# idiap/IdiapTTS

Hardware: AMD Instinct MI355X
Metric: acoustic frames/sec (train) (higher is better)
Workload: dtype f32

## Files before the change

### idiaptts_amd/csrc/sparse_rows.hip

```cpp
#include <algorithm>
#include <atomic>
#include <utility>

#include "activations.h"
#include "common.h"
#include "dropout.h"

namespace itts {

constexpr int kSparseMaxK = 512;
constexpr int kSlabCols = 64;
constexpr int kFwdWaves = 16;
constexpr int kRowsPerWave = 4;
constexpr int kStep = 8;
constexpr int kFetch = 16;
constexpr int kFillTrips = kSparseMaxK / 4 / kFwdWaves;

static std::atomic<int64_t> g_sparse_path[3];

struct ListLayout {
  int64_t counts_off, entries_off, pitch, bytes;
};

static ListLayout list_layout(int64_t M, int K) {
  ListLayout l;
  l.counts_off = 16;
  l.entries_off = 16 + (M * 4 + 15) / 16 * 16;
  l.pitch = ((int64_t)K + kFetch - 1) / kFetch * kFetch;
  l.bytes = l.entries_off + M * l.pitch * 8;
  return l;
}

__global__ __launch_bounds__(256) void sparse_rows_build_kernel(const uint32_t* __restrict__ x, int64_t ldx, int64_t M,
                                                                int K, int* __restrict__ counts,
                                                                int2* __restrict__ entries, int64_t pitch,
                                                                unsigned long long* __restrict__ record) {
  const int lane = threadIdx.x & 63;
  const int64_t w0 = (int64_t)blockIdx.x * 4 + (threadIdx.x >> 6), wn = (int64_t)gridDim.x * 4;
  const unsigned long long below = (1ull << lane) - 1ull;
  unsigned long long total = 0, most = 0;
  for (int64_t m = w0; m < M; m += wn) {
    const uint32_t* row = x + m * ldx;
    int2* out = entries + m * pitch;
    int cnt = 0;
    for (int k0 = 0; k0 < K; k0 += 256) {
      uint32_t bits[4];
#pragma unroll
      for (int u = 0; u < 4; ++u) {
        const int k = k0 + 64 * u + lane;
        bits[u] = k < K ? row[k] : 0u;
      }
#pragma unroll
      for (int u = 0; u < 4; ++u) {
        const bool nz = (bits[u] & 0x7fffffffu) != 0u;
        const unsigned long long mask = __ballot(nz);
        if (nz) out[cnt + __popcll(mask & below)] = make_int2(k0 + 64 * u + lane, (int)bits[u]);
        cnt += __popcll(mask);
      }
    }
    if (lane < ((kStep - cnt % kStep) % kStep)) out[cnt + lane] = make_int2(K, 0);
    if (lane == 0) counts[m] = cnt;
    total += (unsigned long long)cnt;
    most = std::max(most, (unsigned long long)cnt);
  }
  if (record && lane == 0 && total) {
    atomicAdd(&record[0], total);
    atomicMax(&record[1], most);
  }
}

template <int J>
__device__ __forceinline__ void walk_slot(const float4* slab4, int i16, int2 e, float4& acc) {
  const int k = __builtin_amdgcn_update_dpp(0, e.x, 0x150 + J, 0xf, 0xf, false);
  const float v = __int_as_float(__builtin_amdgcn_update_dpp(0, e.y, 0x150 + J, 0xf, 0xf, false));
  const float4 wk = slab4[k * (kSlabCols / 4) + i16];
  acc.x = fmaf(v, wk.x, acc.x); acc.y = fmaf(v, wk.y, acc.y);
  acc.z = fmaf(v, wk.z, acc.z); acc.w = fmaf(v, wk.w, acc.w);
}
template <int FIRST, int... U>
__device__ __forceinline__ void walk_trip(const float4* slab4, int i16, int2 e, float4& acc,
                                          std::integer_sequence<int, U...>) {
  (walk_slot<FIRST + U>(slab4, i16, e, acc), ...);
}

template <int AF, class DR = NoDrop>
__global__ __launch_bounds__(kFwdWaves * 64) void sparse_linear_fwd_kernel(
    const int* __restrict__ counts, const int2* __restrict__ entries, int64_t pitch, const float* __restrict__ w,
    const float* __restrict__ bias, float* __restrict__ y, int64_t ldy, int64_t M, int N, int K, int act, int ranges,
    int store_cols, int wide_out, int wide_w, DR dr) {
  extern __shared__ float4 slab4[];
  float* slab = reinterpret_cast<float*>(slab4);
  const int lane = threadIdx.x & 63;
  const int wave = __builtin_amdgcn_readfirstlane((int)(threadIdx.x >> 6));
  const int n0 = (int)(blockIdx.x / ranges) * kSlabCols;
  const int range = (int)(blockIdx.x % ranges);
  const int64_t per = (M + ranges - 1) / ranges;
  const int64_t m_begin = range * per, m_end = std::min<int64_t>(M, m_begin + per);
  const int q = lane >> 4, c4 = (lane & 15) * 4;

  {
    const bool col_ok = n0 + lane < N;
    const float* wr = w + (int64_t)(col_ok ? n0 + lane : 0) * K;
    if (wide_w) {
      const float4* wr4 = reinterpret_cast<const float4*>(wr);
      const int K4 = K >> 2;
      float4 v[kFillTrips];
#pragma unroll
      for (int u = 0; u < kFillTrips; ++u) {
        const int j = wave + u * kFwdWaves;
        v[u] = (col_ok && j < K4) ? wr4[j] : make_float4(0.f, 0.f, 0.f, 0.f);
      }
#pragma unroll
      for (int u = 0; u < kFillTrips; ++u) {
        const int j = wave + u * kFwdWaves;
        if (j < K4) {
          float* row = slab + 4 * j * kSlabCols + lane;
          row[0] = v[u].x; row[kSlabCols] = v[u].y; row[2 * kSlabCols] = v[u].z; row[3 * kSlabCols] = v[u].w;
        }
      }
    } else {
      for (int k = wave; k < K; k += kFwdWaves) slab[k * kSlabCols + lane] = col_ok ? wr[k] : 0.f;
    }
    if (wave == 0) slab[K * kSlabCols + lane] = 0.f;
  }

  auto row_of = [&](int64_t group) { return m_begin + (group * kRowsPerWave + q); };
  const int i16 = lane & 15;
  auto fetch = [&](int64_t m, int j0) { return entries[std::min<int64_t>(m, M - 1) * pitch + (j0 + i16)]; };
  int64_t group = wave;
  int2 first = fetch(row_of(group), 0);
  int cnt_next = counts[std::min<int64_t>(row_of(group), M - 1)];
  __syncthreads();

  float4 bv = make_float4(0.f, 0.f, 0.f, 0.f);
  const int n = n0 + c4;
  if (bias) {
    if (n < N) bv.x = bias[n];
    if (n + 1 < N) bv.y = bias[n + 1];
    if (n + 2 < N) bv.z = bias[n + 2];
    if (n + 3 < N) bv.w = bias[n + 3];
  }
  const bool vec_store = wide_out && n + 4 <= store_cols;
  const int last_fetch = (int)pitch - kFetch;

  for (; m_begin + group * kRowsPerWave < m_end; group += kFwdWaves) {
    const int64_t m = row_of(group);
    const int cnt = m < m_end ? cnt_next : 0;
    int2 cur = first;
    first = fetch(row_of(group + kFwdWaves), 0);
    cnt_next = counts[std::min<int64_t>(row_of(group + kFwdWaves), M - 1)];
    int longest = std::max(cnt, __shfl_xor(cnt, 16, 64));
    longest = __builtin_amdgcn_readfirstlane(std::max(longest, __shfl_xor(longest, 32, 64)));
    float4 acc = make_float4(0.f, 0.f, 0.f, 0.f);
    for (int j0 = 0; j0 < longest; j0 += kFetch) {
      const int2 nxt = fetch(m, std::min(j0 + kFetch, last_fetch));
      if (j0 < cnt) walk_trip<0>(slab4, i16, cur, acc, std::make_integer_sequence<int, kStep>());
      if (j0 + kStep < cnt) walk_trip<kStep>(slab4, i16, cur, acc, std::make_integer_sequence<int, kStep>());
      cur = nxt;
    }
    if (m < m_end) {
      float4 o;
      o.x = n < N ? act_fwd_af<AF>(acc.x + bv.x, act) : 0.f;
      o.y = n + 1 < N ? act_fwd_af<AF>(acc.y + bv.y, act) : 0.f;
      o.z = n + 2 < N ? act_fwd_af<AF>(acc.z + bv.z, act) : 0.f;
      o.w = n + 3 < N ? act_fwd_af<AF>(acc.w + bv.w, act) : 0.f;
      if constexpr (DR::on) {
        const uint4x dw = dr.words(m, n);
        o.x = dr.apply(o.x, dw.w[0]); o.y = dr.apply(o.y, dw.w[1]);
        o.z = dr.apply(o.z, dw.w[2]); o.w = dr.apply(o.w, dw.w[3]);
      }
      float* yr = y + m * ldy + n;
      if (vec_store) {
        *reinterpret_cast<float4*>(yr) = o;
      } else {
        if (n < store_cols) yr[0] = o.x;
        if (n + 1 < store_cols) yr[1] = o.y;
        if (n + 2 < store_cols) yr[2] = o.z;
        if (n + 3 < store_cols) yr[3] = o.w;
      }
    }
  }
}

}

using namespace itts;

extern "C" int itts_sparse_rows_layout(int64_t M, int K, int64_t out[4]) {
  ITTS_REQUIRE(out != nullptr, "null pointer");
  ITTS_REQUIRE(M >= 0 && K > 0 && K <= 65535, "bad sizes (K <= 65535)");
  const ListLayout l = list_layout(M, K);
  out[0] = l.counts_off; out[1] = l.entries_off; out[2] = l.pitch; out[3] = l.bytes;
  return ITTS_OK;
}

extern "C" int itts_sparse_rows_build(const float* d_x, int64_t ldx, int64_t M, int K, void* d_lists, int want_record,
                                      void* stream) {
  ITTS_REQUIRE(d_lists && (M == 0 || d_x), "null pointer");
  ITTS_REQUIRE(M >= 0 && K > 0 && K <= 65535 && ldx >= K, "bad sizes (K <= 65535)");
  ITTS_REQUIRE(aligned16(d_lists), "the list block must be 16-byte aligned");
  hipStream_t s = as_stream(stream);
  char* base = static_cast<char*>(d_lists);
  if (want_record) ITTS_HIP_CHECK(hipMemsetAsync(base, 0, 16, s));
  if (M == 0) return ITTS_OK;
  const ListLayout l = list_layout(M, K);
  const unsigned grid = (unsigned)std::min<int64_t>((M + 3) / 4, 8192);
  hipLaunchKernelGGL(sparse_rows_build_kernel, dim3(grid), dim3(256), 0, s, reinterpret_cast<const uint32_t*>(d_x), ldx,
                     M, K, reinterpret_cast<int*>(base + l.counts_off), reinterpret_cast<int2*>(base + l.entries_off),
                     l.pitch, want_record ? reinterpret_cast<unsigned long long*>(base) : nullptr);
  ITTS_LAUNCH_CHECK();
  g_sparse_path[0].fetch_add(1, std::memory_order_relaxed);
  return ITTS_OK;
}

static int fwd_compute_units() {
  static int cus = 0;
  if (cus == 0) {
    int dev = 0, n = 0;
    if (hipGetDevice(&dev) != hipSuccess ||
        hipDeviceGetAttribute(&n, hipDeviceAttributeMultiprocessorCount, dev) != hipSuccess || n <= 0)
      n = 256;
    cus = n;
  }
  return cus;
}

template <int AF, class DR = NoDrop>
static int launch_sparse_fwd(const void* d_lists, const float* d_w, const float* d_b, float* d_y, int64_t ldy, int64_t M,
                             int N, int K, int act, hipStream_t s, const DR& dr = DR()) {
  ITTS_HIP_CHECK(itts::allow_dynamic_lds((const void*)sparse_linear_fwd_kernel<AF, DR>, (kSparseMaxK + 1) * kSlabCols * 4));
  const ListLayout l = list_layout(M, K);
  const char* base = static_cast<const char*>(d_lists);
  const int slabs = (N + kSlabCols - 1) / kSlabCols;
  const int64_t ranges = std::max<int64_t>(1, std::min<int64_t>(fwd_compute_units() / slabs, (M + 63) / 64));
  const bool wide_out = (ldy % 4 == 0) && aligned16(d_y);
  const int store_cols = wide_out ? (int)std::min<int64_t>((N + 3) / 4 * 4, ldy) : N;
  hipLaunchKernelGGL((sparse_linear_fwd_kernel<AF, DR>), dim3((unsigned)(slabs * ranges)), dim3(kFwdWaves * 64),
                     (size_t)(K + 1) * kSlabCols * 4, s, reinterpret_cast<const int*>(base + l.counts_off),
                     reinterpret_cast<const int2*>(base + l.entries_off), l.pitch, d_w, d_b, d_y, ldy, M, N, K, act,
                     (int)ranges, store_cols, wide_out ? 1 : 0, (K % 4 == 0 && aligned16(d_w)) ? 1 : 0, dr);
  ITTS_LAUNCH_CHECK();
  return ITTS_OK;
}

template <class DR>
static int linear_fwd_sparse(const void* d_lists, const float* d_x, int64_t ldx, const float* d_w, const float* d_b,
                             float* d_y, int64_t ldy, int64_t M, int N, int K, int act, hipStream_t s, const DR& dr) {
  const char* const entry = DR::on ? "itts_linear_fwd_sparse_dropout" : "itts_linear_fwd_sparse";
  ITTS_REQUIRE_AS(entry, d_w && (M == 0 || (d_lists && d_x && d_y)), "null pointer");
  ITTS_REQUIRE_AS(entry, M >= 0 && N > 0 && K > 0 && K <= 65535 && ldx >= K && ldy >= N, "bad sizes");
  ITTS_REQUIRE_AS(entry, act >= ITTS_ACT_NONE && act <= ITTS_ACT_HARDSIGMOID, "unknown activation");
  if (M == 0) return ITTS_OK;
  if (K > kSparseMaxK) {
    g_sparse_path[2].fetch_add(1, std::memory_order_relaxed);
    return itts::linear_fwd(d_x, ldx, d_w, d_b, d_y, ldy, M, N, K, act, s, dr);
  }
  g_sparse_path[1].fetch_add(1, std::memory_order_relaxed);
  if (act_family(act) == AF_EXT) return launch_sparse_fwd<AF_EXT, DR>(d_lists, d_w, d_b, d_y, ldy, M, N, K, act, s, dr);
  return launch_sparse_fwd<AF_BASE, DR>(d_lists, d_w, d_b, d_y, ldy, M, N, K, act, s, dr);
}

extern "C" int itts_linear_fwd_sparse(const void* d_lists, const float* d_x, int64_t ldx, const float* d_w,
                                      const float* d_b, float* d_y, int64_t ldy, int64_t M, int N, int K, int act,
                                      void* stream) {
  return linear_fwd_sparse(d_lists, d_x, ldx, d_w, d_b, d_y, ldy, M, N, K, act, as_stream(stream), NoDrop{});
}

extern "C" int itts_linear_fwd_sparse_dropout(const void* d_lists, const float* d_x, int64_t ldx, const float* d_w,
                                              const float* d_b, float* d_y, int64_t ldy, int64_t M, int N, int K,
                                              int act, double p, uint64_t seed, uint32_t salt, int64_t row_offset,
                                              void* stream) {
  ITTS_REQUIRE_DROP_P(p);
  if (p == 0.0)
    return linear_fwd_sparse(d_lists, d_x, ldx, d_w, d_b, d_y, ldy, M, N, K, act, as_stream(stream), NoDrop{});
  return linear_fwd_sparse(d_lists, d_x, ldx, d_w, d_b, d_y, ldy, M, N, K, act, as_stream(stream),
                           make_drop_rule(p, seed, salt, row_offset));
}

extern "C" int itts_sparse_path_counts(int64_t out[3]) {
  ITTS_REQUIRE(out != nullptr, "null pointer");
  for (int i = 0; i < 3; ++i) out[i] = g_sparse_path[i].load(std::memory_order_relaxed);
  return ITTS_OK;
}
```

### idiaptts_amd/csrc/sparse_wgrad.hip

```cpp
#include <algorithm>
#include <atomic>

#include "common.h"

namespace itts {

constexpr int kWgMaxK = 512;
constexpr int kTile = 256;
constexpr int kSlab = 64;
constexpr int kWgWaves = 16;
constexpr int kOwners = 64;
constexpr int kSlots = 8;
constexpr int kStrip = 32;
constexpr int kBlock = 16;
constexpr int kGroup = 4;
constexpr int kHeaderBytes = kSlots * 2;
constexpr int kFirstBytes = kBlock * 8;
constexpr int kOverBytes = (kTile / kBlock - 1) * kBlock * 8;
constexpr int kPlanInv = kStrip + kOwners * kSlots;
constexpr int kPlanInts = kPlanInv + kWgMaxK;
constexpr int kHeavyCode = 0x1000;
constexpr int kRowBytes = kSlab * 4;
constexpr int kBufBytes = (kTile + 1) * kRowBytes;
constexpr int kTPitch = 513;
// ... 99 lines not shown
constexpr int kFromRowsLdsBytes = kLists * kFirstBytes + kTile * kStrip * 4 + kFromRowsWaves * kLists * 4 + kWgMaxK * 4;

__global__ __launch_bounds__(kFromRowsWaves * 64) void sparse_cols_from_rows_kernel(
    const int* __restrict__ counts, const int4* __restrict__ entries2, int64_t pitch2, int64_t M, int K, int tiles,
    const int* __restrict__ plan, uint32_t* __restrict__ strip, char* __restrict__ streams) {
  constexpr int T = kFromRowsWaves * 64;
  extern __shared__ uint4 from_rows_lds[];
  int2* first = reinterpret_cast<int2*>(from_rows_lds);
  uint32_t* tile_strip = reinterpret_cast<uint32_t*>(first + kLists * kBlock);
  uint32_t* words = tile_strip + kTile * kStrip;
  int* inverse = reinterpret_cast<int*>(words + kFromRowsWaves * kLists);
  const int tid = threadIdx.x, lane = tid & 63, l32 = lane & 31;
  const int wave = __builtin_amdgcn_readfirstlane(tid >> 6);
  const int tile = (int)blockIdx.x;
  const int64_t m0 = (int64_t)tile * kTile;
  const int row0 = wave * 2 * kFromRowsPairs + (lane >> 5);

  int code_of_tid = -1;
  if (tid < K) {
    const int code = plan[kPlanInv + tid];
    if ((code >= 0 && code < kLists) || (code >= kHeavyCode && code < kHeavyCode + kStrip - 1)) code_of_tid = code;
  }
  int cnt[kFromRowsPairs];
  int4 head[kFromRowsPairs];
#pragma unroll
  for (int q = 0; q < kFromRowsPairs; ++q) {
    const int64_t m = m0 + row0 + 2 * q;
    const bool in = m < M && l32 < pitch2;
    cnt[q] = in ? std::min(counts[m], (int)(2 * pitch2)) : 0;
    head[q] = in ? entries2[m * pitch2 + l32] : make_int4(-1, 0, -1, 0);
  }

  {
    const uint4 neutral = make_uint4((uint32_t)(kTile * kRowBytes), 0u, (uint32_t)(kTile * kRowBytes), 0u);
    uint4* first4 = reinterpret_cast<uint4*>(first);
    for (int i = tid; i < kLists * kFirstBytes / 16; i += T) first4[i] = neutral;
    uint4* strip4 = reinterpret_cast<uint4*>(tile_strip);
    for (int i = tid; i < kTile * kStrip / 4; i += T) {
      const bool ones = (i & 7) == 7 && m0 + (i >> 3) < M;
      strip4[i] = make_uint4(0u, 0u, 0u, ones ? 0x3f800000u : 0u);
    }
    uint4* words4 = reinterpret_cast<uint4*>(words);
    for (int i = tid; i < kFromRowsWaves * kLists / 4; i += T) words4[i] = make_uint4(0u, 0u, 0u, 0u);
    if (tid < kWgMaxK) inverse[tid] = code_of_tid;
  }
  int most = 0;
#pragma unroll
  for (int q = 0; q < kFromRowsPairs; ++q) {
    if (2 * l32 >= cnt[q]) head[q].x = -1;
    if (2 * l32 + 1 >= cnt[q]) head[q].z = -1;
    most = std::max(most, cnt[q]);
  }
  const bool further = std::max(most, __shfl_xor(most, 32, 64)) > 64;
  __syncthreads();

  uint32_t* my_words = words + wave * kLists;
  auto code_of = [&](int k) { return (unsigned)k < (unsigned)K ? inverse[k] : -1; };
  auto again = [&](int q, int j0) {
    int4 e = j0 + 2 * l32 < cnt[q] ? entries2[(m0 + row0 + 2 * q) * pitch2 + j0 / 2 + l32] : make_int4(-1, 0, -1, 0);
    if (j0 + 2 * l32 + 1 >= cnt[q]) e.z = -1;
    e.x = code_of(e.x);
    e.z = code_of(e.z);
    return e;
  };
  auto mark = [&](int q, int code) {
    if (code >= 0 && code < kLists) atomicOr(&my_words[code], 1u << (2 * q + (lane >> 5)));
  };
  auto place = [&](int q, int code, int value) {
    const int row = 2 * q + (lane >> 5);
    if (code >= 0 && code < kLists) {
      const uint32_t word = my_words[code];
      const int pos = (int)(word >> 16) + __popc(word & ((1u << row) - 1u));
      const int2 out = make_int2((row0 + 2 * q) * kRowBytes, value);
      if (pos < kBlock) first[code * kBlock + pos] = out;
      else if (pos < kTile) *entry_of(streams, tiles, (int64_t)tile * kLists + code, pos) = out;
    } else if (code >= kHeavyCode) {
      tile_strip[(row0 + 2 * q) * kStrip + (code - kHeavyCode)] = (uint32_t)value;
    }
  };

#pragma unroll
  for (int q = 0; q < kFromRowsPairs; ++q) {
    head[q].x = code_of(head[q].x);
    head[q].z = code_of(head[q].z);
  }
#pragma unroll
  for (int q = 0; q < kFromRowsPairs; ++q) {
    mark(q, head[q].x);
    mark(q, head[q].z);
  }
  if (further) {
#pragma unroll
    for (int q = 0; q < kFromRowsPairs; ++q)
      for (int j0 = 64; j0 < cnt[q]; j0 += 64) {
        const int4 e = again(q, j0);
        mark(q, e.x);
        mark(q, e.z);
      }
  }
  __syncthreads();

  if (tid < kLists) {
    int run = 0;
#pragma unroll
    for (int w = 0; w < kFromRowsWaves; ++w) {
      const uint32_t rows_of_wave = words[w * kLists + tid];
      words[w * kLists + tid] = rows_of_wave | ((uint32_t)run << 16);
      run += __popc(rows_of_wave);
    }
    reinterpret_cast<uint16_t*>(streams)[(int64_t)tile * kLists + tid] = (uint16_t)run;
  }
  __syncthreads();

#pragma unroll
  for (int q = 0; q < kFromRowsPairs; ++q) {
    place(q, head[q].x, head[q].y);
    place(q, head[q].z, head[q].w);
  }
  if (further) {
#pragma unroll
    for (int q = 0; q < kFromRowsPairs; ++q)
      for (int j0 = 64; j0 < cnt[q]; j0 += 64) {
        const int4 e = again(q, j0);
        place(q, e.x, e.y);
        place(q, e.z, e.w);
      }
  }
  __syncthreads();

  {
    const uint4* first4 = reinterpret_cast<const uint4*>(first);
    uint4* dst = reinterpret_cast<uint4*>(const_cast<char*>(firsts_of(streams, tiles)) +
                                          (int64_t)tile * kLists * kFirstBytes);
    for (int i = tid; i < kLists * kFirstBytes / 16; i += T) dst[i] = first4[i];
    const uint4* strip4 = reinterpret_cast<const uint4*>(tile_strip);
    uint4* sdst = reinterpret_cast<uint4*>(strip + m0 * kStrip);
    for (int i = tid; i < kTile * kStrip / 4; i += T) sdst[i] = strip4[i];
  }
  {
    const int list = tid & (kLists - 1);
    const uint32_t last = words[(kFromRowsWaves - 1) * kLists + list];
    const int total = (int)(last >> 16) + __popc(last & 0xffffu);
    if (total > kBlock) {
      const int end = (total + kBlock - 1) / kBlock * kBlock;
      for (int e = total + (tid >> 9); e < end; e += T / kLists)
        *entry_of(streams, tiles, (int64_t)tile * kLists + list, e) = make_int2(kTile * kRowBytes, 0);
    }
  }
}

typedef float floatx16 __attribute__((ext_vector_type(16)));

template <int J>
__device__ __forceinline__ void col_slot(const char* buf, int lane_off, int2 e, float4& acc) {
  const int off = __builtin_amdgcn_update_dpp(0, e.x, 0x150 + J, 0xf, 0xf, false);
  const float v = __int_as_float(__builtin_amdgcn_update_dpp(0, e.y, 0x150 + J, 0xf, 0xf, false));
  const float4 d = *reinterpret_cast<const float4*>(buf + off + lane_off);
  acc.x = fmaf(v, d.x, acc.x); acc.y = fmaf(v, d.y, acc.y);
  acc.z = fmaf(v, d.z, acc.z); acc.w = fmaf(v, d.w, acc.w);
}
template <int FIRST>
__device__ __forceinline__ void col_group(const char* buf, int lane_off, int2 e, float4& acc) {
  col_slot<FIRST>(buf, lane_off, e, acc);
  col_slot<FIRST + 1>(buf, lane_off, e, acc);
  col_slot<FIRST + 2>(buf, lane_off, e, acc);
  col_slot<FIRST + 3>(buf, lane_off, e, acc);
}

__global__ __launch_bounds__(kWgWaves * 64) void sparse_wgrad_kernel(
    const float* __restrict__ dz, int64_t lddz, const float* __restrict__ strip, const char* __restrict__ streams,
    const int* __restrict__ plan, float* __restrict__ slabs, int64_t slab_stride, int lddw,
    float* __restrict__ bias_part, int64_t bias_stride, int64_t M, int N, int K, int tiles, int per, int ranges) {
  extern __shared__ float4 smem4[];
  char* smem = reinterpret_cast<char*>(smem4);
  float* smemf = reinterpret_cast<float*>(smem4);
  const int tid = threadIdx.x, lane = tid & 63;
  const int wave = __builtin_amdgcn_readfirstlane(tid >> 6);
  const int i16 = lane & 15, owner = wave * 4 + (lane >> 4);
  const int n0 = (int)(blockIdx.x / ranges) * kSlab;
  const int range = (int)(blockIdx.x % ranges);
  const int t_begin = range * per, t_end = std::min(tiles, t_begin + per);

  if (tid < 128) smemf[((tid >> 6) * kBufBytes + kTile * kRowBytes) / 4 + lane] = 0.f;

  const int srow = tid >> 4, c4 = (tid & 15) * 4, n = n0 + c4;
  auto load_tile = [&](int t, float4 (&st)[4]) {
#pragma unroll
    for (int p = 0; p < 4; ++p) {
      const int64_t m = (int64_t)t * kTile + p * 64 + srow;
      float4 v = make_float4(0.f, 0.f, 0.f, 0.f);
      if (m < M) {
        const float* src = dz + m * lddz + n;
        if (n + 4 <= N) {
          v = *reinterpret_cast<const float4*>(src);
        } else {
          if (n < N) v.x = src[0];
          if (n + 1 < N) v.y = src[1];
          if (n + 2 < N) v.z = src[2];
        }
      }
      st[p] = v;
    }
  };
  auto store_tile = [&](int b, const float4 (&st)[4]) {
#pragma unroll
    for (int p = 0; p < 4; ++p)
      *reinterpret_cast<float4*>(smem + b * kBufBytes + (p * 64 + srow) * kRowBytes + c4 * 4) = st[p];
  };
  const char* firsts = firsts_of(streams, tiles) + i16 * 8;
  const char* overs = overs_of(streams, tiles) + i16 * 8;
  auto lists_of = [&](int t) { return ((int64_t)t * kOwners + owner) * kSlots; };

  float4 acc[kSlots];
#pragma unroll
  for (int c = 0; c < kSlots; ++c) acc[c] = make_float4(0.f, 0.f, 0.f, 0.f);
  floatx16 hacc;
#pragma unroll
  for (int r = 0; r < 16; ++r) hacc[r] = 0.f;

  uint4 hdr;
  int2 first[kSlots];
  auto load_lists = [&](int t) {
    hdr = *reinterpret_cast<const uint4*>(streams + ((int64_t)t * kOwners + owner) * kHeaderBytes);
#pragma unroll
    for (int c = 0; c < kSlots; ++c)
      first[c] = *reinterpret_cast<const int2*>(firsts + (lists_of(t) + c) * kFirstBytes);
  };
  auto count_of = [&](int c) {
    const uint32_t word = c < 2 ? hdr.x : (c < 4 ? hdr.y : (c < 6 ? hdr.z : hdr.w));
    return (int)((word >> ((c & 1) * 16)) & 0xffffu);
  };

  float4 st[4];
  load_tile(t_begin, st);
  load_lists(t_begin);
  store_tile(0, st);
  __syncthreads();

  const int hb = wave >> 3, hr0 = (wave & 7) * 32 + (lane >> 5);
  for (int t = t_begin; t < t_end; ++t) {
    const int b = (t - t_begin) & 1;
    const int tn = std::min(t + 1, t_end - 1);
    const char* buf = smem + b * kBufBytes;
    const char* more = overs + lists_of(t) * kOverBytes;
    int2 over = first[0];
    if (count_of(0) > kBlock) over = *reinterpret_cast<const int2*>(more);
#pragma unroll
    for (int c = 0; c < kSlots; ++c) {
      const int cnt = count_of(c);
      int longest = std::max(cnt, __shfl_xor(cnt, 16, 64));
      longest = __builtin_amdgcn_readfirstlane(std::max(longest, __shfl_xor(longest, 32, 64)));
      int2 over_n = over;
      if (c + 1 < kSlots && count_of(c + 1 < kSlots ? c + 1 : c) > kBlock)
        over_n = *reinterpret_cast<const int2*>(more + (c + 1) * kOverBytes);
      int2 cur = first[c];
      for (int j0 = 0; j0 < longest; j0 += kBlock) {
        const int left = cnt - j0;
        if (left > 0) {
          int2 ahead = over;
          if (left > 2 * kBlock) ahead = *reinterpret_cast<const int2*>(more + c * kOverBytes + (j0 + kBlock) * 8);
          col_group<0>(buf, i16 * 16, cur, acc[c]);
          if (left > kGroup) col_group<kGroup>(buf, i16 * 16, cur, acc[c]);
          if (left > 2 * kGroup) col_group<2 * kGroup>(buf, i16 * 16, cur, acc[c]);
          if (left > 3 * kGroup) col_group<3 * kGroup>(buf, i16 * 16, cur, acc[c]);
          cur = over;
          over = ahead;
        }
      }
      over = over_n;
    }
    load_tile(tn, st);
    {
      const float* a = reinterpret_cast<const float*>(buf) + hr0 * kSlab + hb * 32 + (lane & 31);
      const float* xh = strip + ((int64_t)t * kTile + hr0) * kStrip + (lane & 31);
#pragma unroll
      for (int kk = 0; kk < 16; ++kk)
        hacc = __builtin_amdgcn_mfma_f32_32x32x2f32(a[2 * kk * kSlab], xh[2 * kk * kStrip], hacc, 0, 0, 0);
    }
    store_tile(b ^ 1, st);
    load_lists(tn);
    __syncthreads();
  }

  float hsum[2];
  {
#pragma unroll
    for (int r = 0; r < 16; ++r) smemf[(wave * 16 + r) * 64 + lane] = hacc[r];
    __syncthreads();
#pragma unroll
    for (int rr = 0; rr < 2; ++rr) {
      const int r = 2 * (wave & 7) + rr;
      float s = 0.f;
#pragma unroll
      for (int w = 0; w < 8; ++w) s += smemf[((hb * 8 + w) * 16 + r) * 64 + lane];
      hsum[rr] = s;
    }
    __syncthreads();
  }

  for (int i = tid; i < kBiasFloat + kSlab; i += kWgWaves * 64) smemf[i] = 0.f;
  __syncthreads();
#pragma unroll
  for (int c = 0; c < kSlots; ++c) {
    const int col = plan[kStrip + owner * kSlots + c];
    if (col >= 0 && col < K) {
      smemf[(4 * i16 + 0) * kTPitch + col] = acc[c].x;
      smemf[(4 * i16 + 1) * kTPitch + col] = acc[c].y;
      smemf[(4 * i16 + 2) * kTPitch + col] = acc[c].z;
      smemf[(4 * i16 + 3) * kTPitch + col] = acc[c].w;
    }
  }
  {
    const int h = lane & 31;
    const int hc = h < kStrip - 1 ? plan[h] : -1;
#pragma unroll
    for (int rr = 0; rr < 2; ++rr) {
      const int r = 2 * (wave & 7) + rr;
      const int nl = hb * 32 + 8 * (r / 4) + 4 * (lane >> 5) + (r % 4);
      if (h == kStrip - 1) smemf[kBiasFloat + nl] = hsum[rr];
      else if (hc >= 0 && hc < K) smemf[nl * kTPitch + hc] = hsum[rr];
    }
  }
  __syncthreads();
  for (int nn = wave; nn < kSlab; nn += kWgWaves) {
    if (n0 + nn < N) {
      float* dst = slabs + range * slab_stride + (int64_t)(n0 + nn) * lddw;
      for (int k = lane; k < lddw; k += 64) dst[k] = smemf[nn * kTPitch + k];
    }
  }
  if (bias_part && tid < kSlab && n0 + tid < N)
    bias_part[range * bias_stride + n0 + tid] = smemf[kBiasFloat + tid];
}

static int wgrad_compute_units() {
  static int cus = 0;
  if (cus == 0) {
    int dev = 0, n = 0;
    if (hipGetDevice(&dev) != hipSuccess ||
        hipDeviceGetAttribute(&n, hipDeviceAttributeMultiprocessorCount, dev) != hipSuccess || n <= 0)
      n = 256;
    cus = n;
  }
  return cus;
}

static void wgrad_ranges(int64_t M, int N, int* per, int* ranges) {
  const int64_t tiles = (M + kTile - 1) / kTile;
  const int slabs = (N + kSlab - 1) / kSlab;
  const int64_t want = std::max<int64_t>(1, std::min<int64_t>(wgrad_compute_units() / slabs, tiles));
  *per = (int)((tiles + want - 1) / want);
  *ranges = (int)((tiles + *per - 1) / *per);
}

static bool wgrad_shape_ok(int K, int64_t lddw) { return K <= kWgMaxK && lddw <= kWgMaxK; }

}

using namespace itts;

extern "C" int itts_sparse_cols_plan_ints(void) { return kPlanInts; }

extern "C" int itts_sparse_cols_layout(int64_t M, int K, int64_t out[3]) {
  ITTS_REQUIRE(out != nullptr, "null pointer");
  ITTS_REQUIRE(M >= 0 && K > 0 && K <= kWgMaxK, "bad sizes (K <= 512)");
  const ColsLayout l = cols_layout(M);
  out[0] = l.strip_off; out[1] = l.streams_off; out[2] = l.bytes;
  return ITTS_OK;
}

extern "C" int itts_sparse_cols_build(const float* d_x, int64_t ldx, int64_t M, int K, const int* d_plan, void* d_cols,
                                      void* stream) {
  ITTS_REQUIRE(d_plan && d_cols && (M == 0 || d_x), "null pointer");
  ITTS_REQUIRE(M >= 0 && K > 0 && K <= kWgMaxK && ldx >= K, "bad sizes (K <= 512)");
  ITTS_REQUIRE(aligned16(d_cols), "the column block must be 16-byte aligned");
  if (M == 0) return ITTS_OK;
  const ColsLayout l = cols_layout(M);
  const int parts = (K + 63) / 64;
  ITTS_REQUIRE(l.tiles * (parts + 1) < ((int64_t)1 << 31), "too many rows");
  char* base = static_cast<char*>(d_cols);
  hipLaunchKernelGGL(sparse_cols_build_kernel, dim3((unsigned)(l.tiles * (parts + 1))), dim3(256), 0,
                     as_stream(stream), reinterpret_cast<const uint32_t*>(d_x), ldx, M, K, parts, (int)l.tiles, d_plan,
                     reinterpret_cast<uint32_t*>(base + l.strip_off), base + l.streams_off);
  ITTS_LAUNCH_CHECK();
  g_wgrad_path[0].fetch_add(1, std::memory_order_relaxed);
  return ITTS_OK;
}

extern "C" int itts_sparse_cols_build_from_rows(const void* d_lists, int64_t M, int K_lists, int K, const int* d_plan,
                                                void* d_cols, void* stream) {
  ITTS_REQUIRE(d_plan && d_cols && (M == 0 || d_lists), "null pointer");
  ITTS_REQUIRE(M >= 0 && K > 0 && K <= kWgMaxK && K_lists >= K && K_lists <= 65535,
               "bad sizes (K <= 512, K <= K_lists <= 65535)");
  ITTS_REQUIRE(aligned16(d_cols) && aligned16(d_lists), "the column and list blocks must be 16-byte aligned");
  if (M == 0) return ITTS_OK;
  int64_t rows[4];
  if (int rc = itts_sparse_rows_layout(M, K_lists, rows)) return rc;
  const ColsLayout l = cols_layout(M);
  ITTS_REQUIRE(l.tiles < ((int64_t)1 << 31), "too many rows");
  ITTS_HIP_CHECK(itts::allow_dynamic_lds((const void*)sparse_cols_from_rows_kernel, kFromRowsLdsBytes));
  const char* lists = static_cast<const char*>(d_lists);
  char* base = static_cast<char*>(d_cols);
  hipLaunchKernelGGL(sparse_cols_from_rows_kernel, dim3((unsigned)l.tiles), dim3(kFromRowsWaves * 64),
                     kFromRowsLdsBytes, as_stream(stream), reinterpret_cast<const int*>(lists + rows[0]),
                     reinterpret_cast<const int4*>(lists + rows[1]), rows[2] / 2, M, K, (int)l.tiles, d_plan,
                     reinterpret_cast<uint32_t*>(base + l.strip_off), base + l.streams_off);
  ITTS_LAUNCH_CHECK();
  g_wgrad_path[0].fetch_add(1, std::memory_order_relaxed);
  return ITTS_OK;
}

extern "C" int64_t itts_linear_bwd_weight_sparse_workspace_bytes(int64_t M, int N, int K, int64_t lddw) {
  if (M < 0 || N <= 0 || K <= 0 || lddw < K) return 0;
  const int64_t dense = itts_linear_bwd_weight_workspace_bytes(M, N, (int)lddw);
  if (M == 0 || !wgrad_shape_ok(K, lddw)) return dense;
  int per, ranges;
  wgrad_ranges(M, N, &per, &ranges);
  return std::max<int64_t>(dense, (int64_t)ranges * ((int64_t)N * lddw + N) * 4);
// ... 45 lines not shown
```

Measured before the change: 43.41 million.

## Sort sparse rows by nonzero count per wave block to balance forward walks

The sparse forward kernel now gives each wave a contiguous share of rows, processed in blocks of 64. Within each block, rows are bucket-sorted by nonzero count using ballots and ds_permute, so the four rows sharing a wave step have similar lengths and less of the wave sits idle. The inner walk is split into 4-entry half-trips that batch their LDS reads before the packed FMAs. It also pins waves_per_eu and swaps update_dpp for mov_dpp with a hoisted lane offset in both the forward and wgrad kernels. The ranking adds per-block overhead, and the new row partitioning changes load balance across waves.

```diff
diff --git a/idiaptts_amd/csrc/sparse_rows.hip b/idiaptts_amd/csrc/sparse_rows.hip
--- a/idiaptts_amd/csrc/sparse_rows.hip
+++ b/idiaptts_amd/csrc/sparse_rows.hip
@@ -12,8 +12,12 @@
 constexpr int kSlabCols = 64;
 constexpr int kFwdWaves = 16;
 constexpr int kRowsPerWave = 4;
+constexpr int kBlockRows = 64;
 constexpr int kStep = 8;
+constexpr int kHalf = 4;
 constexpr int kFetch = 16;
+constexpr int kRankBuckets = 8;
+static_assert(kStep % kHalf == 0 && kFetch % kHalf == 0, "half-trips tile the padded lists and the fetches");
 constexpr int kFillTrips = kSparseMaxK / 4 / kFwdWaves;
 
 static std::atomic<int64_t> g_sparse_path[3];
@@ -69,22 +73,77 @@
   }
 }
 
-template <int J>
-__device__ __forceinline__ void walk_slot(const float4* slab4, int i16, int2 e, float4& acc) {
-  const int k = __builtin_amdgcn_update_dpp(0, e.x, 0x150 + J, 0xf, 0xf, false);
-  const float v = __int_as_float(__builtin_amdgcn_update_dpp(0, e.y, 0x150 + J, 0xf, 0xf, false));
-  const float4 wk = slab4[k * (kSlabCols / 4) + i16];
-  acc.x = fmaf(v, wk.x, acc.x); acc.y = fmaf(v, wk.y, acc.y);
-  acc.z = fmaf(v, wk.z, acc.z); acc.w = fmaf(v, wk.w, acc.w);
-}
-template <int FIRST, int... U>
-__device__ __forceinline__ void walk_trip(const float4* slab4, int i16, int2 e, float4& acc,
-                                          std::integer_sequence<int, U...>) {
-  (walk_slot<FIRST + U>(slab4, i16, e, acc), ...);
+template <int CTRL>
+__device__ __forceinline__ int dpp_mov(int v) {
+  return __builtin_amdgcn_mov_dpp(v, CTRL, 0xf, 0xf, true);
+}
+constexpr int kDppQuadSwap1 = 0xb1, kDppQuadSwap2 = 0x4e;
+constexpr int kDppRowHalfMirror = 0x141, kDppRowMirror = 0x140, kDppRowBcast = 0x150;
+
+typedef float floatx2 __attribute__((ext_vector_type(2)));
+typedef float floatx4 __attribute__((ext_vector_type(4)));
+struct WalkAcc {
+  floatx2 lo, hi;
+};
+template <int FIRST>
+__device__ __forceinline__ int walk_bcast(int x, int u) {
+  static_assert(kHalf == 4, "one case per slot of a half-trip");
+  switch (u) {
+    case 0: return dpp_mov<kDppRowBcast + FIRST>(x);
+    case 1: return dpp_mov<kDppRowBcast + FIRST + 1>(x);
+    case 2: return dpp_mov<kDppRowBcast + FIRST + 2>(x);
+    default: return dpp_mov<kDppRowBcast + FIRST + 3>(x);
+  }
+}
+template <int FIRST>
+__device__ __forceinline__ floatx4 walk_read(const char* slab_lane, int kb, int u) {
+  return *reinterpret_cast<const floatx4*>(slab_lane + walk_bcast<FIRST>(kb, u));
+}
+template <int FIRST>
+__device__ __forceinline__ void walk_half(const char* slab_lane, int kb, int val, WalkAcc& acc) {
+  floatx4 wk[kHalf];
+#pragma unroll
+  for (int u = 0; u < kHalf; ++u) wk[u] = walk_read<FIRST>(slab_lane, kb, u);
+#pragma unroll
+  for (int u = 0; u < kHalf; ++u) {
+    const float v = __int_as_float(walk_bcast<FIRST>(val, u));
+    const floatx2 vv = {v, v};
+    acc.lo = __builtin_elementwise_fma(vv, wk[u].xy, acc.lo);
+    acc.hi = __builtin_elementwise_fma(vv, wk[u].zw, acc.hi);
+  }
+}
+
+__device__ __forceinline__ int wave_min(int x) {
+  x = std::min(x, dpp_mov<kDppQuadSwap1>(x));
+  x = std::min(x, dpp_mov<kDppQuadSwap2>(x));
+  x = std::min(x, dpp_mov<kDppRowHalfMirror>(x));
+  x = std::min(x, dpp_mov<kDppRowMirror>(x));
+  return std::min(std::min(__builtin_amdgcn_readlane(x, 0), __builtin_amdgcn_readlane(x, 16)),
+                  std::min(__builtin_amdgcn_readlane(x, 32), __builtin_amdgcn_readlane(x, 48)));
+}
+
+__device__ __forceinline__ int rank_block(int cnt, bool valid, int lane) {
+  const int key = (int)((unsigned)(cnt + kHalf - 1) / kHalf);
+  const int kmin = wave_min(valid ? key : 0x7fffffff);
+  const int bucket = valid ? std::min(key - kmin, kRankBuckets - 1) : kRankBuckets;
+  int rank = lane, before = 0;
+#pragma unroll
+  for (int b = 0; b < kRankBuckets; ++b) {
+    const unsigned long long mask = __ballot(bucket == b);
+    const int pos = (int)__builtin_amdgcn_mbcnt_hi((uint32_t)(mask >> 32),
+                                                   __builtin_amdgcn_mbcnt_lo((uint32_t)mask, (uint32_t)before));
+    rank = bucket == b ? pos : rank;
+    before += __popcll(mask);
+  }
+  const int sorted = __builtin_amdgcn_ds_permute(rank << 2, (key << 16) | (cnt << 6) | lane);
+  int longest = sorted >> 16;
+  longest = std::max(longest, dpp_mov<kDppQuadSwap1>(longest));
+  longest = std::max(longest, dpp_mov<kDppQuadSwap2>(longest));
+  return (longest << 16) | (sorted & 0xffff);
 }
 
 template <int AF, class DR = NoDrop>
-__global__ __launch_bounds__(kFwdWaves * 64) void sparse_linear_fwd_kernel(
+__global__ __launch_bounds__(kFwdWaves * 64) __attribute__((amdgpu_waves_per_eu(4, 4))) void sparse_linear_fwd_kernel(
     const int* __restrict__ counts, const int2* __restrict__ entries, int64_t pitch, const float* __restrict__ w,
     const float* __restrict__ bias, float* __restrict__ y, int64_t ldy, int64_t M, int N, int K, int act, int ranges,
     int store_cols, int wide_out, int wide_w, DR dr) {
@@ -124,12 +183,19 @@
     if (wave == 0) slab[K * kSlabCols + lane] = 0.f;
   }
 
-  auto row_of = [&](int64_t group) { return m_begin + (group * kRowsPerWave + q); };
+  const int64_t share = std::max<int64_t>(kBlockRows, (m_end - m_begin + kBlockRows - 1) / kBlockRows * kRowsPerWave);
+  const int64_t w_begin = m_begin + wave * share, w_end = std::min(m_end, w_begin + share);
   const int i16 = lane & 15;
   auto fetch = [&](int64_t m, int j0) { return entries[std::min<int64_t>(m, M - 1) * pitch + (j0 + i16)]; };
-  int64_t group = wave;
-  int2 first = fetch(row_of(group), 0);
-  int cnt_next = counts[std::min<int64_t>(row_of(group), M - 1)];
+  auto block_begin = [&](int64_t b) { return w_begin + b * kBlockRows; };
+  auto count_of_lane = [&](int64_t b) {
+    const int64_t m = block_begin(b) + lane;
+    const int c = counts[std::min<int64_t>(m, M - 1)];
+    return m < w_end ? c : 0;
+  };
+  auto group_of = [&](int sorted, int g) { return __builtin_amdgcn_ds_bpermute((g * kRowsPerWave + q) << 2, sorted); };
+  int64_t block = 0;
+  int cnt_next = count_of_lane(block);
   __syncthreads();
 
   float4 bv = make_float4(0.f, 0.f, 0.f, 0.f);
@@ -143,27 +209,53 @@
   const bool vec_store = wide_out && n + 4 <= store_cols;
   const int last_fetch = (int)pitch - kFetch;
 
-  for (; m_begin + group * kRowsPerWave < m_end; group += kFwdWaves) {
-    const int64_t m = row_of(group);
-    const int cnt = m < m_end ? cnt_next : 0;
+  if (block_begin(block) >= w_end) return;
+  const char* slab_lane = reinterpret_cast<const char*>(slab4) + i16 * 16;
+  auto groups_of = [&](int64_t b) {
+    const int64_t rows = std::min<int64_t>(kBlockRows, w_end - block_begin(b));
+    return (int)((rows + kRowsPerWave - 1) / kRowsPerWave);
+  };
+  int sorted = rank_block(cnt_next, block_begin(block) + lane < w_end, lane);
+  cnt_next = count_of_lane(block + 1);
+  int groups = groups_of(block), g = 0;
+  int item = group_of(sorted, g);
+  int2 first = fetch(block_begin(block) + (item & 63), 0);
+
+  for (;;) {
+    const int cnt = (item >> 6) & 1023;
+    const int longest = __builtin_amdgcn_readfirstlane(item >> 16) * kHalf;
+    const int64_t m = block_begin(block) + (item & 63);
     int2 cur = first;
-    first = fetch(row_of(group + kFwdWaves), 0);
-    cnt_next = counts[std::min<int64_t>(row_of(group + kFwdWaves), M - 1)];
-    int longest = std::max(cnt, __shfl_xor(cnt, 16, 64));
-    longest = __builtin_amdgcn_readfirstlane(std::max(longest, __shfl_xor(longest, 32, 64)));
-    float4 acc = make_float4(0.f, 0.f, 0.f, 0.f);
+    bool more = true;
+    if (++g == groups) {
+      block += 1;
+      g = 0;
+      more = block_begin(block) < w_end;
+      if (more) {
+        sorted = rank_block(cnt_next, block_begin(block) + lane < w_end, lane);
+        cnt_next = count_of_lane(block + 1);
+        groups = groups_of(block);
+      }
+    }
+    item = group_of(sorted, g);
+    first = fetch(block_begin(block) + (item & 63), 0);
+
+    WalkAcc acc = {{0.f, 0.f}, {0.f, 0.f}};
     for (int j0 = 0; j0 < longest; j0 += kFetch) {
       const int2 nxt = fetch(m, std::min(j0 + kFetch, last_fetch));
-      if (j0 < cnt) walk_trip<0>(slab4, i16, cur, acc, std::make_integer_sequence<int, kStep>());
-      if (j0 + kStep < cnt) walk_trip<kStep>(slab4, i16, cur, acc, std::make_integer_sequence<int, kStep>());
+      const int kb = cur.x * (kSlabCols * 4);
+      if (j0 < cnt) walk_half<0>(slab_lane, kb, cur.y, acc);
+      if (j0 + kHalf < cnt) walk_half<kHalf>(slab_lane, kb, cur.y, acc);
+      if (j0 + 2 * kHalf < cnt) walk_half<2 * kHalf>(slab_lane, kb, cur.y, acc);
+      if (j0 + 3 * kHalf < cnt) walk_half<3 * kHalf>(slab_lane, kb, cur.y, acc);
       cur = nxt;
     }
-    if (m < m_end) {
+    if (m < w_end) {
       float4 o;
-      o.x = n < N ? act_fwd_af<AF>(acc.x + bv.x, act) : 0.f;
-      o.y = n + 1 < N ? act_fwd_af<AF>(acc.y + bv.y, act) : 0.f;
-      o.z = n + 2 < N ? act_fwd_af<AF>(acc.z + bv.z, act) : 0.f;
-      o.w = n + 3 < N ? act_fwd_af<AF>(acc.w + bv.w, act) : 0.f;
+      o.x = n < N ? act_fwd_af<AF>(acc.lo.x + bv.x, act) : 0.f;
+      o.y = n + 1 < N ? act_fwd_af<AF>(acc.lo.y + bv.y, act) : 0.f;
+      o.z = n + 2 < N ? act_fwd_af<AF>(acc.hi.x + bv.z, act) : 0.f;
+      o.w = n + 3 < N ? act_fwd_af<AF>(acc.hi.y + bv.w, act) : 0.f;
       if constexpr (DR::on) {
         const uint4x dw = dr.words(m, n);
         o.x = dr.apply(o.x, dw.w[0]); o.y = dr.apply(o.y, dw.w[1]);
@@ -179,6 +271,7 @@
         if (n + 3 < store_cols) yr[3] = o.w;
       }
     }
+    if (!more) break;
   }
 }
 
diff --git a/idiaptts_amd/csrc/sparse_wgrad.hip b/idiaptts_amd/csrc/sparse_wgrad.hip
--- a/idiaptts_amd/csrc/sparse_wgrad.hip
+++ b/idiaptts_amd/csrc/sparse_wgrad.hip
@@ -275,19 +275,19 @@
 typedef float floatx16 __attribute__((ext_vector_type(16)));
 
 template <int J>
-__device__ __forceinline__ void col_slot(const char* buf, int lane_off, int2 e, float4& acc) {
-  const int off = __builtin_amdgcn_update_dpp(0, e.x, 0x150 + J, 0xf, 0xf, false);
-  const float v = __int_as_float(__builtin_amdgcn_update_dpp(0, e.y, 0x150 + J, 0xf, 0xf, false));
-  const float4 d = *reinterpret_cast<const float4*>(buf + off + lane_off);
+__device__ __forceinline__ void col_slot(const char* buf_lane, int2 e, float4& acc) {
+  const int off = __builtin_amdgcn_mov_dpp(e.x, 0x150 + J, 0xf, 0xf, true);
+  const float v = __int_as_float(__builtin_amdgcn_mov_dpp(e.y, 0x150 + J, 0xf, 0xf, true));
+  const float4 d = *reinterpret_cast<const float4*>(buf_lane + off);
   acc.x = fmaf(v, d.x, acc.x); acc.y = fmaf(v, d.y, acc.y);
   acc.z = fmaf(v, d.z, acc.z); acc.w = fmaf(v, d.w, acc.w);
 }
 template <int FIRST>
-__device__ __forceinline__ void col_group(const char* buf, int lane_off, int2 e, float4& acc) {
-  col_slot<FIRST>(buf, lane_off, e, acc);
-  col_slot<FIRST + 1>(buf, lane_off, e, acc);
-  col_slot<FIRST + 2>(buf, lane_off, e, acc);
-  col_slot<FIRST + 3>(buf, lane_off, e, acc);
+__device__ __forceinline__ void col_group(const char* buf_lane, int2 e, float4& acc) {
+  col_slot<FIRST>(buf_lane, e, acc);
+  col_slot<FIRST + 1>(buf_lane, e, acc);
+  col_slot<FIRST + 2>(buf_lane, e, acc);
+  col_slot<FIRST + 3>(buf_lane, e, acc);
 }
 
 __global__ __launch_bounds__(kWgWaves * 64) void sparse_wgrad_kernel(
@@ -365,6 +365,7 @@
     const int b = (t - t_begin) & 1;
     const int tn = std::min(t + 1, t_end - 1);
     const char* buf = smem + b * kBufBytes;
+    const char* buf_lane = buf + i16 * 16;
     const char* more = overs + lists_of(t) * kOverBytes;
     int2 over = first[0];
     if (count_of(0) > kBlock) over = *reinterpret_cast<const int2*>(more);
@@ -382,10 +383,10 @@
         if (left > 0) {
           int2 ahead = over;
           if (left > 2 * kBlock) ahead = *reinterpret_cast<const int2*>(more + c * kOverBytes + (j0 + kBlock) * 8);
-          col_group<0>(buf, i16 * 16, cur, acc[c]);
-          if (left > kGroup) col_group<kGroup>(buf, i16 * 16, cur, acc[c]);
-          if (left > 2 * kGroup) col_group<2 * kGroup>(buf, i16 * 16, cur, acc[c]);
-          if (left > 3 * kGroup) col_group<3 * kGroup>(buf, i16 * 16, cur, acc[c]);
+          col_group<0>(buf_lane, cur, acc[c]);
+          if (left > kGroup) col_group<kGroup>(buf_lane, cur, acc[c]);
+          if (left > 2 * kGroup) col_group<2 * kGroup>(buf_lane, cur, acc[c]);
+          if (left > 3 * kGroup) col_group<3 * kGroup>(buf_lane, cur, acc[c]);
           cur = over;
           over = ahead;
         }
```

Measured after the change: 43.35 million. No clear change (-0.1%).

## Prefetch three entry fetches per row ahead and store via buffer ops in sparse forward

Applied to the files above, without the earlier changes.

The sparse forward kernel now issues the count and the first three 16-entry fetches for the next row group with inline-asm global loads, then waits on them explicitly with vmcnt so that list loads overlap the current row's LDS walk. Rows with at most 48 entries need no serial fetch chain. Slab offsets are precomputed in bytes, the DPP bound_ctrl flag is set, and wide outputs use a buffer-resource store with out-of-range masking instead of a branch. This aims to hide global latency on the entry lists, at the cost of fragile hand-written waitcnt assumptions and extra registers.

```diff
diff --git a/idiaptts_amd/csrc/sparse_rows.hip b/idiaptts_amd/csrc/sparse_rows.hip
--- a/idiaptts_amd/csrc/sparse_rows.hip
+++ b/idiaptts_amd/csrc/sparse_rows.hip
@@ -14,7 +14,14 @@
 constexpr int kRowsPerWave = 4;
 constexpr int kStep = 8;
 constexpr int kFetch = 16;
+constexpr int kAhead = 48;
+constexpr int kAheadFetches = kAhead / kFetch;
+constexpr int kSlabRowBytes = kSlabCols * 4;
 constexpr int kFillTrips = kSparseMaxK / 4 / kFwdWaves;
+static_assert(kAhead % kFetch == 0 && kFetch == 2 * kStep, "the walk takes a fetch as two trips");
+
+typedef float floatx4 __attribute__((ext_vector_type(4)));
+typedef int intx2 __attribute__((ext_vector_type(2)));
 
 static std::atomic<int64_t> g_sparse_path[3];
 
@@ -70,17 +77,22 @@
 }
 
 template <int J>
-__device__ __forceinline__ void walk_slot(const float4* slab4, int i16, int2 e, float4& acc) {
-  const int k = __builtin_amdgcn_update_dpp(0, e.x, 0x150 + J, 0xf, 0xf, false);
-  const float v = __int_as_float(__builtin_amdgcn_update_dpp(0, e.y, 0x150 + J, 0xf, 0xf, false));
-  const float4 wk = slab4[k * (kSlabCols / 4) + i16];
+__device__ __forceinline__ void walk_slot(const char* slab, int lane_off, int2 e, float4& acc) {
+  const int off = __builtin_amdgcn_update_dpp(0, e.x, 0x150 + J, 0xf, 0xf, true);
+  const float v = __int_as_float(__builtin_amdgcn_update_dpp(0, e.y, 0x150 + J, 0xf, 0xf, true));
+  const float4 wk = *reinterpret_cast<const float4*>(slab + (off + lane_off));
   acc.x = fmaf(v, wk.x, acc.x); acc.y = fmaf(v, wk.y, acc.y);
   acc.z = fmaf(v, wk.z, acc.z); acc.w = fmaf(v, wk.w, acc.w);
 }
 template <int FIRST, int... U>
-__device__ __forceinline__ void walk_trip(const float4* slab4, int i16, int2 e, float4& acc,
+__device__ __forceinline__ void walk_trip(const char* slab, int lane_off, int2 e, float4& acc,
                                           std::integer_sequence<int, U...>) {
-  (walk_slot<FIRST + U>(slab4, i16, e, acc), ...);
+  (walk_slot<FIRST + U>(slab, lane_off, e, acc), ...);
+}
+__device__ __forceinline__ int2 slab_offsets(int2 e) { return make_int2(e.x * kSlabRowBytes, e.y); }
+__device__ __forceinline__ void walk_fetch(const char* slab, int lane_off, int2 e, int left, float4& acc) {
+  if (left > 0) walk_trip<0>(slab, lane_off, e, acc, std::make_integer_sequence<int, kStep>());
+  if (left > kStep) walk_trip<kStep>(slab, lane_off, e, acc, std::make_integer_sequence<int, kStep>());
 }
 
 template <int AF, class DR = NoDrop>
@@ -126,10 +138,34 @@
 
   auto row_of = [&](int64_t group) { return m_begin + (group * kRowsPerWave + q); };
   const int i16 = lane & 15;
-  auto fetch = [&](int64_t m, int j0) { return entries[std::min<int64_t>(m, M - 1) * pitch + (j0 + i16)]; };
+  const int last_fetch = (int)pitch - kFetch;
+  auto fetch = [&](int64_t m, int j0) {
+    return entries[std::min<int64_t>(m, M - 1) * pitch + (std::min(j0, last_fetch) + i16)];
+  };
+  struct Ahead {
+    int cnt;
+    intx2 e[kAheadFetches];
+  };
+  static_assert(kAheadFetches == 3, "request_ahead and wait_ahead name three fetches");
+  auto request_ahead = [&](int64_t group, Ahead& a) {
+    const int64_t m = std::min<int64_t>(row_of(group), M - 1);
+    const int* pc = counts + m;
+    const int2* pe = entries + m * pitch + i16;
+    const int2 *p0 = pe, *p1 = pe + std::min(kFetch, last_fetch), *p2 = pe + std::min(2 * kFetch, last_fetch);
+    asm volatile("global_load_dword %0, %1, off" : "=v"(a.cnt) : "v"(pc) : "memory");
+    asm volatile("global_load_dwordx2 %0, %1, off" : "=v"(a.e[0]) : "v"(p0) : "memory");
+    asm volatile("global_load_dwordx2 %0, %1, off" : "=v"(a.e[1]) : "v"(p1) : "memory");
+    asm volatile("global_load_dwordx2 %0, %1, off" : "=v"(a.e[2]) : "v"(p2) : "memory");
+  };
+  auto wait_ahead = [&](auto keep, Ahead& a) {
+    asm volatile("s_nop 1\n\ts_waitcnt vmcnt(%4)"
+                 : "+v"(a.cnt), "+v"(a.e[0]), "+v"(a.e[1]), "+v"(a.e[2])
+                 : "n"(decltype(keep)::value)
+                 : "memory");
+  };
   int64_t group = wave;
-  int2 first = fetch(row_of(group), 0);
-  int cnt_next = counts[std::min<int64_t>(row_of(group), M - 1)];
+  Ahead next;
+  request_ahead(group, next);
   __syncthreads();
 
   float4 bv = make_float4(0.f, 0.f, 0.f, 0.f);
@@ -140,25 +176,46 @@
     if (n + 2 < N) bv.z = bias[n + 2];
     if (n + 3 < N) bv.w = bias[n + 3];
   }
-  const bool vec_store = wide_out && n + 4 <= store_cols;
-  const int last_fetch = (int)pitch - kFetch;
-
-  for (; m_begin + group * kRowsPerWave < m_end; group += kFwdWaves) {
-    const int64_t m = row_of(group);
-    const int cnt = m < m_end ? cnt_next : 0;
-    int2 cur = first;
-    first = fetch(row_of(group + kFwdWaves), 0);
-    cnt_next = counts[std::min<int64_t>(row_of(group + kFwdWaves), M - 1)];
-    int longest = std::max(cnt, __shfl_xor(cnt, 16, 64));
-    longest = __builtin_amdgcn_readfirstlane(std::max(longest, __shfl_xor(longest, 32, 64)));
-    float4 acc = make_float4(0.f, 0.f, 0.f, 0.f);
-    for (int j0 = 0; j0 < longest; j0 += kFetch) {
-      const int2 nxt = fetch(m, std::min(j0 + kFetch, last_fetch));
-      if (j0 < cnt) walk_trip<0>(slab4, i16, cur, acc, std::make_integer_sequence<int, kStep>());
-      if (j0 + kStep < cnt) walk_trip<kStep>(slab4, i16, cur, acc, std::make_integer_sequence<int, kStep>());
-      cur = nxt;
-    }
-    if (m < m_end) {
+  const char* slab_bytes = reinterpret_cast<const char*>(slab4);
+  const int lane_off = i16 * 16;
+  asm volatile("" ::"v"(bv.x), "v"(bv.y), "v"(bv.z), "v"(bv.w));
+  wait_ahead(std::integral_constant<int, 0>{}, next);
+
+  auto run = [&](auto wide) {
+    constexpr bool WIDE = decltype(wide)::value;
+    const int64_t range_rows = std::max<int64_t>(m_end - m_begin, 1);
+    const __amdgpu_buffer_rsrc_t yrs = __builtin_amdgcn_make_buffer_rsrc(
+        y + m_begin * ldy, 0, WIDE ? (int)(((range_rows - 1) * ldy + store_cols) * 4) : 0, 0x00020000);
+    for (; m_begin + group * kRowsPerWave < m_end; group += kFwdWaves) {
+      const int64_t m = row_of(group);
+      const Ahead cur = next;
+      request_ahead(group + kFwdWaves, next);
+      const int cnt = m < m_end ? cur.cnt : 0;
+      int longest = std::max(cnt, __shfl_xor(cnt, 16, 64));
+      longest = __builtin_amdgcn_readfirstlane(std::max(longest, __shfl_xor(longest, 32, 64)));
+      float4 acc = make_float4(0.f, 0.f, 0.f, 0.f);
+      auto walk_ahead = [&]() {
+#pragma unroll
+        for (int f = 0; f < kAheadFetches; ++f)
+          if (f * kFetch < longest)
+            walk_fetch(slab_bytes, lane_off, slab_offsets(make_int2(cur.e[f].x, cur.e[f].y)), cnt - f * kFetch, acc);
+      };
+      if (longest <= kAhead) {
+        walk_ahead();
+      } else {
+        auto landed = [](int2 e) { asm volatile("" ::"v"(e.x), "v"(e.y)); };
+        int2 more = fetch(m, kAhead);
+        walk_ahead();
+        int j0 = kAhead;
+        for (; j0 + kFetch < longest; j0 += kFetch) {
+          const int2 nxt = fetch(m, j0 + kFetch);
+          landed(more);
+          walk_fetch(slab_bytes, lane_off, slab_offsets(more), cnt - j0, acc);
+          more = nxt;
+        }
+        landed(more);
+        walk_fetch(slab_bytes, lane_off, slab_offsets(more), cnt - j0, acc);
+      }
       float4 o;
       o.x = n < N ? act_fwd_af<AF>(acc.x + bv.x, act) : 0.f;
       o.y = n + 1 < N ? act_fwd_af<AF>(acc.y + bv.y, act) : 0.f;
@@ -169,17 +226,26 @@
         o.x = dr.apply(o.x, dw.w[0]); o.y = dr.apply(o.y, dw.w[1]);
         o.z = dr.apply(o.z, dw.w[2]); o.w = dr.apply(o.w, dw.w[3]);
       }
-      float* yr = y + m * ldy + n;
-      if (vec_store) {
-        *reinterpret_cast<float4*>(yr) = o;
+      if constexpr (WIDE) {
+        const bool stores = m < m_end && n + 4 <= store_cols;
+        const uint32_t vo = stores ? (uint32_t)(((m - m_begin) * ldy + n) * 4) : 0xfffffff0u;
+        floatx4 ov = {o.x, o.y, o.z, o.w};
+        __builtin_amdgcn_raw_buffer_store_b128(ov, yrs, vo, 0, 0);
+        wait_ahead(std::integral_constant<int, 1>{}, next);
       } else {
+        if (m < m_end) {
+        float* yr = y + m * ldy + n;
         if (n < store_cols) yr[0] = o.x;
         if (n + 1 < store_cols) yr[1] = o.y;
         if (n + 2 < store_cols) yr[2] = o.z;
         if (n + 3 < store_cols) yr[3] = o.w;
+        }
+        wait_ahead(std::integral_constant<int, 0>{}, next);
       }
     }
-  }
+  };
+  if (wide_out) run(std::true_type{});
+  else run(std::false_type{});
 }
 
 }
@@ -232,8 +298,9 @@
   const ListLayout l = list_layout(M, K);
   const char* base = static_cast<const char*>(d_lists);
   const int slabs = (N + kSlabCols - 1) / kSlabCols;
-  const int64_t ranges = std::max<int64_t>(1, std::min<int64_t>(fwd_compute_units() / slabs, (M + 63) / 64));
-  const bool wide_out = (ldy % 4 == 0) && aligned16(d_y);
+  int64_t ranges = std::max<int64_t>(1, std::min<int64_t>(fwd_compute_units() / slabs, (M + 63) / 64));
+  const bool wide_out = (ldy % 4 == 0) && aligned16(d_y) && ldy < (int64_t(1) << 28);
+  if (wide_out) ranges = std::max(ranges, (M * ldy * 4 >> 31) + 1);
   const int store_cols = wide_out ? (int)std::min<int64_t>((N + 3) / 4 * 4, ldy) : N;
   hipLaunchKernelGGL((sparse_linear_fwd_kernel<AF, DR>), dim3((unsigned)(slabs * ranges)), dim3(kFwdWaves * 64),
                      (size_t)(K + 1) * kSlabCols * 4, s, reinterpret_cast<const int*>(base + l.counts_off),
diff --git a/idiaptts_amd/csrc/sparse_wgrad.hip b/idiaptts_amd/csrc/sparse_wgrad.hip
--- a/idiaptts_amd/csrc/sparse_wgrad.hip
+++ b/idiaptts_amd/csrc/sparse_wgrad.hip
@@ -276,8 +276,8 @@
 
 template <int J>
 __device__ __forceinline__ void col_slot(const char* buf, int lane_off, int2 e, float4& acc) {
-  const int off = __builtin_amdgcn_update_dpp(0, e.x, 0x150 + J, 0xf, 0xf, false);
-  const float v = __int_as_float(__builtin_amdgcn_update_dpp(0, e.y, 0x150 + J, 0xf, 0xf, false));
+  const int off = __builtin_amdgcn_update_dpp(0, e.x, 0x150 + J, 0xf, 0xf, true);
+  const float v = __int_as_float(__builtin_amdgcn_update_dpp(0, e.y, 0x150 + J, 0xf, 0xf, true));
   const float4 d = *reinterpret_cast<const float4*>(buf + off + lane_off);
   acc.x = fmaf(v, d.x, acc.x); acc.y = fmaf(v, d.y, acc.y);
   acc.z = fmaf(v, d.z, acc.z); acc.w = fmaf(v, d.w, acc.w);
```

Result: faster. 43.65 million before, 44.63 million after, median of 6 (+2.3%).
